# pothosware/PothosComms

Measured on NVIDIA B200. Metric: FIR Msamples/s (cf32, 256 taps) at 1/2/4/8 B200; % HBM roofline; vs host CPU, higher is better.
Workload: dtype f32

## Files before the change

pothoscomms_b200/csrc/fir_os.cu:

```cuda
#include <algorithm>
#include <cmath>
#include <complex>
#include <cstdlib>
#include <vector>

#include "bulk.cuh"
#include "fft.hpp"
#include "os64_core.cuh"

namespace b200c {

struct FirOs64Args {
    const void *in;
    void *out;
    const void *hf;
    const void *twa;
    const void *twb;
    const void *twf;
    long long n_in;
    long long n_out;
    long long in_stride, out_stride;
    int nchan;
    int K;
    int parts;
};

template <bool CONJ, bool SLOT_REV>
__device__ __forceinline__ void step_twiddle(c2 (&v)[64], const c2 *__restrict__ twa, const c2 *__restrict__ twb, const int t)
{
    c2 A[8], B[8];
#pragma unroll
    for (int i = 1; i < 8; i++) { A[i] = twa[i * 64 + t]; B[i] = twb[i * 64 + t]; }
#pragma unroll
    for (int a = 0; a < 8; a++)
#pragma unroll
        for (int b = 0; b < 8; b++) {
            const int j = 8 * a + b, r = SLOT_REV ? rev64(j) : j;
            if (a) v[r] = cmul_p<CONJ>(v[r], A[a]);
            if (b) v[r] = cmul_p<CONJ>(v[r], B[b]);
        }
}

constexpr int kBulkElems = 4098;

template <int MINB>
__global__ void __launch_bounds__(64, MINB) fir_os64_kernel(const FirOs64Args a)
{
    __shared__ __align__(16) c2 F[kOs64SmemElems];
    __shared__ __align__(8) unsigned long long bar;
    const int t = threadIdx.x;
    const c2 *__restrict__ twa = static_cast<const c2 *>(a.twa);
    const c2 *__restrict__ twb = static_cast<const c2 *>(a.twb);
    const int Km1 = a.K - 1;
    const int hop = 4096 - Km1;
    const long long nblk = (a.n_out + hop - 1) / hop;
    const long long tstep = gridDim.x, dch = tstep / nblk, dblk = tstep - dch * nblk;
    long long ch = (long long)blockIdx.x / nblk, blk = (long long)blockIdx.x - ch * nblk;
    auto bulk_src = [&](long long ch, long long blk, const c2 *&src) {
        if (ch >= a.nchan) return false;
        const long long base = blk * hop;
        const c2 *in = static_cast<const c2 *>(a.in) + ch * a.in_stride;
        const int mis = (int)(((reinterpret_cast<unsigned long long>(in) >> 3) + base) & 1);
        src = in + (base - mis);
        return base - mis >= 0 && base - mis + kBulkElems <= a.n_in;
    };
    if (t == 0) mbar_init(&bar, 1);
    __syncthreads();
    const c2 *src = nullptr;
    bool pending = bulk_src(ch, blk, src);
    if (pending && t == 0) bulk_load(F, src, kBulkElems * (unsigned)sizeof(c2), &bar);
    unsigned parity = 0;

    while (ch < a.nchan) {
        const long long base = blk * hop;
        long long nch = ch + dch, nblkpos = blk + dblk;
        if (nblkpos >= nblk) { nblkpos -= nblk; nch++; }
        const c2 *__restrict__ in = static_cast<const c2 *>(a.in) + ch * a.in_stride;
        const c2 *__restrict__ hf = static_cast<const c2 *>(a.hf) + ch * 4096;
        c2 *__restrict__ out = static_cast<c2 *>(a.out) + ch * a.out_stride;
        c2 v[64];
        if (pending) {
            const int mis = (int)(((reinterpret_cast<unsigned long long>(in) >> 3) + base) & 1);
            mbar_wait(&bar, parity);
            parity ^= 1;
#pragma unroll
            for (int n1 = 0; n1 < 64; n1++) v[rev64(n1)] = F[mis + 64 * n1 + t];
        } else {
#pragma unroll
            for (int n1 = 0; n1 < 64; n1++) {
                const long long g = base + 64 * n1 + t;
                v[rev64(n1)] = g < a.n_in ? __ldcg(in + g) : 0ull;
            }
        }
        dft64_dit<false>(v);
        step_twiddle<false, false>(v, twa, twb, t);
        __syncthreads();
#pragma unroll
        for (int k1 = 0; k1 < 64; k1++) F[k1 * kOs64Stride + t] = v[k1];
        __syncthreads();
#pragma unroll
        for (int n2 = 0; n2 < 64; n2++) v[rev64(n2)] = F[t * kOs64Stride + n2];
        dft64_dit<false>(v);
#pragma unroll
        for (int k2 = 0; k2 < 64; k2++) v[k2] = cmul_p<false>(v[k2], hf[64 * k2 + t]);
        dft64_dif<true>(v);
        step_twiddle<true, true>(v, twa, twb, t);
        __syncthreads();
#pragma unroll
        for (int n2 = 0; n2 < 64; n2++) F[t * kOs64Stride + n2] = v[rev64(n2)];
        __syncthreads();
#pragma unroll
        for (int k1 = 0; k1 < 64; k1++) v[k1] = F[k1 * kOs64Stride + t];
        __syncthreads();
        pending = bulk_src(nch, nblkpos, src);
        if (pending && t == 0) bulk_load(F, src, kBulkElems * (unsigned)sizeof(c2), &bar);
        dft64_dif<true>(v);
        c2 *o = out + (base - Km1);
        if (base + hop <= a.n_out) {
#pragma unroll
            for (int n1 = 0; n1 < 64; n1++) {
                const int i = 64 * n1 + t;
                if (i >= Km1) __stcg(o + i, v[rev64(n1)]);
            }
        } else {
#pragma unroll
            for (int n1 = 0; n1 < 64; n1++) {
                const int i = 64 * n1 + t;
                if (i >= Km1 && base + i - Km1 < a.n_out) __stcg(o + i, v[rev64(n1)]);
            }
        }
        ch = nch; blk = nblkpos;
    }
}

constexpr int kOs64Groups = 4;
__global__ void __launch_bounds__(64 * kOs64Groups, 1) fir_os64p_kernel(const FirOs64Args a)
{
    extern __shared__ __align__(16) c2 os64p_dyn[];
    __shared__ __align__(8) unsigned long long bars[kOs64Groups];
    const int g = threadIdx.x >> 6, t = threadIdx.x & 63;
    c2 *F = os64p_dyn + g * kOs64SmemElems;
    c2 *TW = os64p_dyn + kOs64Groups * kOs64SmemElems;
    c2 *HF = TW + 4096;
    unsigned long long *bar = &bars[g];
    auto gsync = [&] { asm volatile("bar.sync %0, 64;" ::"r"(g + 1) : "memory"); };
    const int Km1 = a.K - 1;
    const int hop = 4096 - Km1;
    const long long nblk = (a.n_out + hop - 1) / hop;
    const long long parts = a.parts, ntask = (long long)a.nchan * parts;
    const long long bstep = parts * kOs64Groups;
    auto bulk_src = [&](long long ch, long long blk, const c2 *&src) {
        if (ch >= a.nchan || blk >= nblk) return false;
        const long long base = blk * hop;
        const c2 *in = static_cast<const c2 *>(a.in) + ch * a.in_stride;
        const int mis = (int)(((reinterpret_cast<unsigned long long>(in) >> 3) + base) & 1);
        src = in + (base - mis);
        return base - mis >= 0 && base - mis + kBulkElems <= a.n_in;
    };
    long long task = blockIdx.x;
    if (t == 0) mbar_init(bar, 1);
    gsync();
    const c2 *src = nullptr;
    bool pending = task < ntask && bulk_src(task / parts, (task % parts) * kOs64Groups + g, src);
    if (pending && t == 0) bulk_load(F, src, kBulkElems * (unsigned)sizeof(c2), bar);
    unsigned parity = 0;
    {
        const c2 *__restrict__ twf = static_cast<const c2 *>(a.twf);
        for (int i = threadIdx.x; i < 4096; i += 64 * kOs64Groups) TW[i] = twf[i];
    }
    long long staged = -1;
    for (; task < ntask; task += gridDim.x) {
        const long long ch = task / parts, first = (task - ch * parts) * kOs64Groups + g;
        if (ch != staged) {
            const c2 *__restrict__ hfg = static_cast<const c2 *>(a.hf) + ch * 4096;
            for (int i = threadIdx.x; i < 4096; i += 64 * kOs64Groups) HF[i] = __ldg(hfg + i);
            staged = ch;
        }
        __syncthreads();
        const c2 *__restrict__ in = static_cast<const c2 *>(a.in) + ch * a.in_stride;
        c2 *__restrict__ out = static_cast<c2 *>(a.out) + ch * a.out_stride;
        for (long long blk = first; blk < nblk; blk += bstep) {
            const long long base = blk * hop;
            c2 v[64];
            if (pending) {
                const int mis = (int)(((reinterpret_cast<unsigned long long>(in) >> 3) + base) & 1);
                mbar_wait(bar, parity);
                parity ^= 1;
#pragma unroll
                for (int n1 = 0; n1 < 64; n1++) v[rev64(n1)] = F[mis + 64 * n1 + t];
            } else {
#pragma unroll
                for (int n1 = 0; n1 < 64; n1++) {
                    const long long gi = base + 64 * n1 + t;
                    v[rev64(n1)] = gi < a.n_in ? __ldcg(in + gi) : 0ull;
                }
            }
            dft64_dit<false>(v);
#pragma unroll
            for (int k1 = 1; k1 < 64; k1++) v[k1] = cmul_p<false>(v[k1], TW[k1 * 64 + t]);
            gsync();
#pragma unroll
            for (int k1 = 0; k1 < 64; k1++) F[k1 * kOs64Stride + t] = v[k1];
            gsync();
#pragma unroll
            for (int n2 = 0; n2 < 64; n2++) v[rev64(n2)] = F[t * kOs64Stride + n2];
            dft64_dit<false>(v);
#pragma unroll
            for (int k2 = 0; k2 < 64; k2++) v[k2] = cmul_p<false>(v[k2], HF[64 * k2 + t]);
            dft64_dif<true>(v);
#pragma unroll
            for (int n2 = 1; n2 < 64; n2++) v[rev64(n2)] = cmul_p<true>(v[rev64(n2)], TW[n2 * 64 + t]);
            gsync();
#pragma unroll
            for (int n2 = 0; n2 < 64; n2++) F[t * kOs64Stride + n2] = v[rev64(n2)];
            gsync();
#pragma unroll
            for (int k1 = 0; k1 < 64; k1++) v[k1] = F[k1 * kOs64Stride + t];
            gsync();
            {
                const bool last = blk + bstep >= nblk;
                const long long nt = task + gridDim.x;
                pending = last ? (nt < ntask && bulk_src(nt / parts, (nt % parts) * kOs64Groups + g, src)) : bulk_src(ch, blk + bstep, src);
                if (pending && t == 0) bulk_load(F, src, kBulkElems * (unsigned)sizeof(c2), bar);
            }
            dft64_dif<true>(v);
            c2 *o = out + (base - Km1);
            if (base + hop <= a.n_out) {
#pragma unroll
                for (int n1 = 0; n1 < 64; n1++) {
                    const int i = 64 * n1 + t;
                    if (i >= Km1) __stcg(o + i, v[rev64(n1)]);
                }
            } else {
#pragma unroll
                for (int n1 = 0; n1 < 64; n1++) {
                    const int i = 64 * n1 + t;
                    if (i >= Km1 && base + i - Km1 < a.n_out) __stcg(o + i, v[rev64(n1)]);
                }
            }
        }
        __syncthreads();
    }
}


constexpr bool kOs32PartialTwiddles = false;

template <bool CONJ, bool SLOT_REV>
__device__ __forceinline__ void twiddle32(c2 (&v)[32], const c2 *__restrict__ tw, const int t)
{
    c2 A[8], B[4];
#pragma unroll
    for (int a = 1; a < 8; a++) A[a] = tw[(4 * a) * 32 + t];
#pragma unroll
    for (int b = 1; b < 4; b++) B[b] = tw[b * 32 + t];
#pragma unroll
    for (int k = 1; k < 32; k++) {
        const int a = k >> 2, b = k & 3, r = SLOT_REV ? rev32(k) : k;
        if (a) v[r] = cmul_p<CONJ>(v[r], A[a]);
        if (b) v[r] = cmul_p<CONJ>(v[r], B[b]);
    }
}

struct FirOs32Args {
    const void *in;
    void *out;
    const void *hf;
    const void *tw;
    long long n_in, n_out;
    long long in_stride, out_stride;
    int nchan;
    int K;
    int spread;
    int pdl;
};

constexpr int kOs32Landing = 1032;
template <int WARPS, int MINB, bool TABS = false, bool PT = kOs32PartialTwiddles, bool EARLY = false>
__global__ void __launch_bounds__(32 * WARPS, MINB) fir_os32_kernel(const FirOs32Args a)
{
    extern __shared__ __align__(16) c2 os32_dyn[];
    __shared__ __align__(16) c2 Fs[TABS ? 1 : WARPS][TABS ? 1 : kOs32SmemElems];
    __shared__ __align__(8) unsigned long long bars[WARPS];
    const int t = threadIdx.x & 31, w = threadIdx.x >> 5;
    c2 *F = TABS ? os32_dyn + w * kOs32SmemElems : Fs[TABS ? 0 : w];
    unsigned long long *bar = &bars[w];
    const c2 *__restrict__ tw = static_cast<const c2 *>(a.tw);
    const c2 *__restrict__ hf_tab = nullptr;
    c2 *Lb = F;
    if constexpr (TABS && EARLY) Lb = os32_dyn + WARPS * kOs32SmemElems + 2048 + w * kOs32Landing;
    const int Km1 = a.K - 1;
    const int hop = 1024 - Km1;
    const long long nblk = (a.n_out + hop - 1) / hop;
    const long long tstep = (long long)gridDim.x * WARPS, dch = tstep / nblk, dblk = tstep - dch * nblk;
    const long long task0 = a.spread ? (long long)w * gridDim.x + blockIdx.x : (long long)blockIdx.x * WARPS + w;
    long long ch = task0 / nblk, blk = task0 - ch * nblk;
    constexpr int kBulk = 1026;
    auto bulk_src = [&](long long ch, long long blk, const c2 *&src) {
        if (ch >= a.nchan) return false;
        const long long base = blk * hop;
        const c2 *in = static_cast<const c2 *>(a.in) + ch * a.in_stride;
        const int mis = (int)(((reinterpret_cast<unsigned long long>(in) >> 3) + base) & 1);
        src = in + (base - mis);
        return base - mis >= 0 && base - mis + kBulk <= a.n_in;
    };
    if (t == 0) mbar_init(bar, 1);
    __syncwarp();
    const c2 *src = nullptr;
    bool pending = bulk_src(ch, blk, src);
    unsigned parity = 0;
    if constexpr (TABS) {
        asm volatile("griddepcontrol.launch_dependents;");
        c2 *tab = os32_dyn + WARPS * kOs32SmemElems;
        const c2 *__restrict__ hf0 = static_cast<const c2 *>(a.hf);
        if (a.pdl) {
            for (int i = threadIdx.x; i < 1024; i += 32 * WARPS) { tab[i] = hf0[i]; tab[1024 + i] = tw[i]; }
            asm volatile("griddepcontrol.wait;" ::: "memory");
            if (pending && t == 0) bulk_load(Lb, src, kBulk * (unsigned)sizeof(c2), bar);
        } else {
            if (pending && t == 0) bulk_load(Lb, src, kBulk * (unsigned)sizeof(c2), bar);
            for (int i = threadIdx.x; i < 1024; i += 32 * WARPS) { tab[i] = hf0[i]; tab[1024 + i] = tw[i]; }
        }
        __syncthreads();
        hf_tab = tab; tw = tab + 1024;
    } else {
        if (pending && t == 0) bulk_load(Lb, src, kBulk * (unsigned)sizeof(c2), bar);
    }
    while (ch < a.nchan) {
        const long long base = blk * hop;
        long long nch = ch + dch, nblkpos = blk + dblk;
        if (nblkpos >= nblk) { nblkpos -= nblk; nch++; }
        const c2 *__restrict__ in = static_cast<const c2 *>(a.in) + ch * a.in_stride;
        const c2 *__restrict__ hf = TABS ? hf_tab : static_cast<const c2 *>(a.hf) + ch * 1024;
        c2 *__restrict__ out = static_cast<c2 *>(a.out) + ch * a.out_stride;
        c2 v[32];
        if (pending) {
            const int mis = (int)(((reinterpret_cast<unsigned long long>(in) >> 3) + base) & 1);
            mbar_wait(bar, parity);
            parity ^= 1;
#pragma unroll
            for (int n1 = 0; n1 < 32; n1++) v[rev32(n1)] = Lb[mis + 32 * n1 + t];
        } else {
#pragma unroll
            for (int n1 = 0; n1 < 32; n1++) {
                const long long g = base + 32 * n1 + t;
                v[rev32(n1)] = g < a.n_in ? __ldcg(in + g) : 0ull;
            }
        }
        if constexpr (TABS && EARLY) {
            __syncwarp();
            pending = bulk_src(nch, nblkpos, src);
            if (pending && t == 0) bulk_load(Lb, src, kBulk * (unsigned)sizeof(c2), bar);
        }
        dft32_dit<false>(v);
        if constexpr (PT) twiddle32<false, false>(v, tw, t);
        else {
#pragma unroll
            for (int k1 = 1; k1 < 32; k1++) v[k1] = cmul_p<false>(v[k1], tw[k1 * 32 + t]);
        }
        __syncwarp();
#pragma unroll
        for (int k1 = 0; k1 < 32; k1++) F[k1 * kOs32Stride + t] = v[k1];
        __syncwarp();
#pragma unroll
        for (int n2 = 0; n2 < 32; n2++) v[rev32(n2)] = F[t * kOs32Stride + n2];
        dft32_dit<false>(v);
#pragma unroll
        for (int k2 = 0; k2 < 32; k2++) v[k2] = cmul_p<false>(v[k2], hf[32 * k2 + t]);
        dft32_dif<true>(v);
        if constexpr (PT) twiddle32<true, true>(v, tw, t);
        else {
#pragma unroll
            for (int n2 = 1; n2 < 32; n2++) v[rev32(n2)] = cmul_p<true>(v[rev32(n2)], tw[n2 * 32 + t]);
        }
        __syncwarp();
#pragma unroll
        for (int n2 = 0; n2 < 32; n2++) F[t * kOs32Stride + n2] = v[rev32(n2)];
        __syncwarp();
#pragma unroll
        for (int k1 = 0; k1 < 32; k1++) v[k1] = F[k1 * kOs32Stride + t];
        if constexpr (!(TABS && EARLY)) {
            __syncwarp();
            pending = bulk_src(nch, nblkpos, src);
            if (pending && t == 0) bulk_load(F, src, kBulk * (unsigned)sizeof(c2), bar);
        }
        dft32_dif<true>(v);
        c2 *o = out + (base - Km1);
        if (base + hop <= a.n_out) {
#pragma unroll
            for (int n1 = 0; n1 < 32; n1++) {
                const int i = 32 * n1 + t;
                if (i >= Km1) __stcg(o + i, v[rev32(n1)]);
            }
        } else {
#pragma unroll
            for (int n1 = 0; n1 < 32; n1++) {
                const int i = 32 * n1 + t;
                if (i >= Km1 && base + i - Km1 < a.n_out) __stcg(o + i, v[rev32(n1)]);
            }
        }
        ch = nch; blk = nblkpos;
    }
}

B200C_HD constexpr float cos48(int e)
{
    constexpr float t[48] = {
        1.0f, 0.9914448857307434f, 0.9659258127212524f, 0.9238795042037964f, 0.8660253882408142f, 0.7933533191680908f,
        0.7071067690849304f, 0.6087614297866821f, 0.5f, 0.3826834261417389f, 0.258819043636322f, 0.13052618503570557f, 0.0f,
        -0.13052618503570557f, -0.258819043636322f, -0.3826834261417389f, -0.5f, -0.6087614297866821f, -0.7071067690849304f,
        -0.7933533191680908f, -0.8660253882408142f, -0.9238795042037964f, -0.9659258127212524f, -0.9914448857307434f, -1.0f,
        -0.9914448857307434f, -0.9659258127212524f, -0.9238795042037964f, -0.8660253882408142f, -0.7933533191680908f,
        -0.7071067690849304f, -0.6087614297866821f, -0.5f, -0.3826834261417389f, -0.258819043636322f, -0.13052618503570557f, 0.0f,
        0.13052618503570557f, 0.258819043636322f, 0.3826834261417389f, 0.5f, 0.6087614297866821f, 0.7071067690849304f,
        0.7933533191680908f, 0.8660253882408142f, 0.9238795042037964f, 0.9659258127212524f, 0.9914448857307434f};
    return t[e % 48];
}
B200C_HD constexpr float sin48(int e) { return cos48(e + 36); }

B200C_HD constexpr int rev16(int k) { return 4 * (k & 3) + (k >> 2); }
template <bool INV> B200C_HD void dft16_dif(c2 (&x)[16])
{
#pragma unroll
    for (int k = 0; k < 4; k++) {
        dft4_p<INV>(x[k], x[k + 4], x[k + 8], x[k + 12]);
        x[k + 4] = mul_w64<INV>(x[k + 4], 4 * k);
        x[k + 8] = mul_w64<INV>(x[k + 8], 8 * k);
        x[k + 12] = mul_w64<INV>(x[k + 12], 12 * k);
    }
#pragma unroll
    for (int g = 0; g < 4; g++) dft4_p<INV>(x[4 * g], x[4 * g + 1], x[4 * g + 2], x[4 * g + 3]);
}

B200C_HD c2 cmul_acc(c2 f, c2 w, c2 acc)
{
    float fx, fy, wx, wy;
    upk(f, fx, fy); upk(w, wx, wy);
    return fma2(f, pk(wx, wx), fma2(pk(-fy, fx), pk(wy, wy), acc));
}

struct FirOsX32Args {
    const void *in;
    void *out;
    const void *hx;
    const void *tw;
    const void *tw3;
    long long n_in, n_out;
    long long p0;
    int m0;
    int pdl;
};
constexpr int kX32Rows = 48, kX32SmemElems = kX32Rows * kOs32Stride;

constexpr int kX32TabElems = 3072 + 1536 + 1024;
template <int WARPS, int MINB, bool PT = false, bool SPLIT = false>
__global__ void __launch_bounds__(32 * WARPS, MINB) fir_os32x_kernel(const FirOsX32Args a)
{
    extern __shared__ __align__(16) c2 x32_smem[];
    __shared__ __align__(8) unsigned long long bars[WARPS];
    const int t = threadIdx.x & 31, wp = threadIdx.x >> 5;
    const c2 *__restrict__ tw = static_cast<const c2 *>(a.tw);
    const c2 *__restrict__ tw3 = static_cast<const c2 *>(a.tw3);
    const c2 *__restrict__ hx = static_cast<const c2 *>(a.hx);
    c2 *F = x32_smem + wp * kX32SmemElems;
    c2 *const Lb = F;
    unsigned long long &bar = bars[wp];
    const c2 *__restrict__ in = static_cast<const c2 *>(a.in);
    c2 *__restrict__ out = static_cast<c2 *>(a.out);
    const int m0 = a.m0, hop_out = 1536 - m0, hop_in = hop_out / 3 * 2;
    const long long nblk = (a.n_out + hop_out - 1) / hop_out;
    constexpr int kBulk = 1026;
    auto bulk_src = [&](long long blk, const c2 *&src) {
        if (blk >= nblk) return false;
        const long long P = a.p0 + blk * hop_in;
        const int mis = (int)(((reinterpret_cast<unsigned long long>(in) >> 3) + (unsigned long long)P) & 1);
        src = in + (P - mis);
        return P - mis >= 0 && P - mis + kBulk <= a.n_in;
    };
    if (t == 0) mbar_init(&bar, 1);
    __syncwarp();
    long long blk = (long long)blockIdx.x * WARPS + wp;
    const long long bstep = (long long)gridDim.x * WARPS;
    const c2 *src = nullptr;
    bool pending = bulk_src(blk, src);
    unsigned parity = 0;
    if constexpr (WARPS > 1) {
        asm volatile("griddepcontrol.launch_dependents;");
        c2 *tab = x32_smem + WARPS * kX32SmemElems;
        auto stage = [&] {
            for (int i = threadIdx.x; i < 3072; i += 32 * WARPS) tab[i] = hx[i];
            for (int i = threadIdx.x; i < 1536; i += 32 * WARPS) tab[3072 + i] = tw3[i];
            for (int i = threadIdx.x; i < 1024; i += 32 * WARPS) tab[3072 + 1536 + i] = tw[i];
        };
        if (a.pdl) {
            stage();
            asm volatile("griddepcontrol.wait;" ::: "memory");
            if (pending && t == 0) bulk_load(Lb, src, kBulk * (unsigned)sizeof(c2), &bar);
        } else {
            if (pending && t == 0) bulk_load(Lb, src, kBulk * (unsigned)sizeof(c2), &bar);
            stage();
        }
        __syncthreads();
        hx = tab; tw3 = tab + 3072; tw = tab + 3072 + 1536;
    } else {
        if (pending && t == 0) bulk_load(Lb, src, kBulk * (unsigned)sizeof(c2), &bar);
    }
    for (; blk < nblk; blk += bstep) {
        const long long P = a.p0 + blk * hop_in;
        c2 v[32];
        if (pending) {
            const int mis = (int)(((reinterpret_cast<unsigned long long>(in) >> 3) + (unsigned long long)P) & 1);
            mbar_wait(&bar, parity);
            parity ^= 1;
#pragma unroll
            for (int n1 = 0; n1 < 32; n1++) v[rev32(n1)] = Lb[mis + 32 * n1 + t];
        } else {
#pragma unroll
            for (int n1 = 0; n1 < 32; n1++) {
                const long long g = P + 32 * n1 + t;
                v[rev32(n1)] = (g >= 0 && g < a.n_in) ? __ldcg(in + g) : 0ull;
            }
        }
        dft32_dit<false>(v);
        if constexpr (PT) twiddle32<false, false>(v, tw, t);
        else {
#pragma unroll
            for (int k1 = 1; k1 < 32; k1++) v[k1] = cmul_p<false>(v[k1], tw[k1 * 32 + t]);
        }
        __syncwarp();
#pragma unroll
        for (int k1 = 0; k1 < 32; k1++) F[k1 * kOs32Stride + t] = v[k1];
        __syncwarp();
#pragma unroll
        for (int n2 = 0; n2 < 32; n2++) v[rev32(n2)] = F[t * kOs32Stride + n2];
        dft32_dit<false>(v);
        c2 s[3][16];
#pragma unroll
        for (int c = 0; c < 16; c++) {
            const c2 xa = v[c], xb = v[c + 16];
            const c2 h0 = hx[32 * c + t], g0 = hx[1536 + 32 * c + t];
            const c2 h1 = hx[32 * (c + 16) + t], g1 = hx[1536 + 32 * (c + 16) + t];
            const c2 h2 = hx[32 * (c + 32) + t], g2 = hx[1536 + 32 * (c + 32) + t];
            s[c % 3][c / 3] = cmul_acc(xb, g0, cmul_p<false>(xa, h0));
            s[(c + 16) % 3][(c + 16) / 3] = cmul_acc(xa, g1, cmul_p<false>(xb, h1));
            s[(c + 32) % 3][(c + 32) / 3] = cmul_acc(xb, g2, cmul_p<false>(xa, h2));
        }
#pragma unroll
        for (int c1 = 0; c1 < 3; c1++) dft16_dif<true>(s[c1]);
        __syncwarp();
        c2 twb1 = 0, twb2 = 0;
        if constexpr (PT) { twb1 = tw3[16 * 32 + t]; twb2 = tw3[32 * 32 + t]; }
#pragma unroll
        for (int v2 = 0; v2 < 16; v2++) {
            const int r = rev16(v2);
            const c2 a0 = s[0][r];
            const c2 a1 = v2 ? cmul_s(s[1][r], cos48(v2), sin48(v2)) : s[1][r];
            const c2 a2 = v2 ? cmul_s(s[2][r], cos48(2 * v2), sin48(2 * v2)) : s[2][r];
            const c2 t1 = add2(a1, a2);
            const c2 t2 = fma2(t1, pk(-0.5f, -0.5f), a0);
            const c2 t3 = rot_p<true>(mul2(sub2(a1, a2), pk(0.8660254037844386f, 0.8660254037844386f)));
            const c2 y0 = add2(a0, t1), y1 = add2(t2, t3), y2 = sub2(t2, t3);
            if constexpr (PT) {
                const c2 wa = v2 ? tw3[v2 * 32 + t] : pk(1.f, 0.f);
                F[v2 * kOs32Stride + t] = v2 ? cmul_p<false>(y0, wa) : y0;
                F[(16 + v2) * kOs32Stride + t] = cmul_p<false>(y1, v2 ? cmul_p<false>(wa, twb1) : twb1);
                F[(32 + v2) * kOs32Stride + t] = cmul_p<false>(y2, v2 ? cmul_p<false>(wa, twb2) : twb2);
            } else {
                F[v2 * kOs32Stride + t] = v2 ? cmul_p<false>(y0, tw3[v2 * 32 + t]) : y0;
                F[(16 + v2) * kOs32Stride + t] = cmul_p<false>(y1, tw3[(16 + v2) * 32 + t]);
                F[(32 + v2) * kOs32Stride + t] = cmul_p<false>(y2, tw3[(32 + v2) * 32 + t]);
            }
        }
        __syncwarp();
        const long long mbase = blk * hop_out - m0;
        const bool whole = (blk + 1) * (long long)hop_out <= a.n_out;
        c2 *const o = out + mbase + t;
        const int d0 = t - m0;
        const int left = whole ? 0x7fffffff : (int)(a.n_out - mbase) - t;
#pragma unroll
        for (int k1 = 0; k1 < 32; k1++) v[rev32(k1)] = F[t * kOs32Stride + k1];
        if constexpr (SPLIT) {
            __syncwarp();
            pending = bulk_src(blk + bstep, src);
            if (pending && t == 0) bulk_load(F, src, kBulk * (unsigned)sizeof(c2), &bar);
        }
        dft32_dit<true>(v);
        if (whole) {
#pragma unroll
            for (int n1 = 0; n1 < 32; n1++)
                if (d0 + 48 * n1 >= 0) __stcg(o + 48 * n1, v[n1]);
        } else {
#pragma unroll
            for (int n1 = 0; n1 < 32; n1++)
                if (d0 + 48 * n1 >= 0 && 48 * n1 < left) __stcg(o + 48 * n1, v[n1]);
        }
        if constexpr (SPLIT) {
            const int tt = t & 15, h = t >> 4;
            c2 x[16];
#pragma unroll
            for (int j = 0; j < 16; j++) x[j] = F[(32 + tt) * kOs32Stride + 2 * j + h];
            __syncwarp();
            dft16_dif<true>(x);
            c2 *const o2 = out + mbase + tt + 32 + 48 * 16 * h;
            const int d2 = tt - m0 + 32 + 48 * 16 * h;
            const int left2 = whole ? 0x7fffffff : (int)(a.n_out - mbase) - tt - 32 - 48 * 16 * h;
#pragma unroll
            for (int m = 0; m < 16; m++) {
                const c2 mine = h ? mul_w64<true>(x[rev16(m)], 2 * m) : x[rev16(m)];
                const c2 other = __shfl_xor_sync(0xffffffffu, mine, 16);
                const c2 y = h ? sub2(other, mine) : add2(mine, other);
                if (d2 + 48 * m >= 0 && 48 * m < left2) __stcg(o2 + 48 * m, y);
            }
            continue;
        }
        if (t < 16) {
#pragma unroll
            for (int k1 = 0; k1 < 32; k1++) v[rev32(k1)] = F[(32 + t) * kOs32Stride + k1];
        }
        __syncwarp();
        pending = bulk_src(blk + bstep, src);
        if (pending && t == 0) bulk_load(F, src, kBulk * (unsigned)sizeof(c2), &bar);
        if (t < 16) {
            dft32_dit<true>(v);
            if (whole) {
#pragma unroll
                for (int n1 = 0; n1 < 32; n1++)
                    if (d0 + 48 * n1 + 32 >= 0) __stcg(o + 48 * n1 + 32, v[n1]);
            } else {
#pragma unroll
                for (int n1 = 0; n1 < 32; n1++)
                    if (d0 + 48 * n1 + 32 >= 0 && 48 * n1 + 32 < left) __stcg(o + 48 * n1 + 32, v[n1]);
            }
        }
    }
}

struct FirOs32RArgs {
    const float *in;
    float *out;
    const void *hf;
    const void *tw;
    long long n_in, n_out;
    int K;
};

template <int WARPS, int MINB, bool EARLY = false>
__global__ void __launch_bounds__(32 * WARPS, MINB) fir_os32r_kernel(const FirOs32RArgs a)
{
    extern __shared__ __align__(16) c2 os32r_dyn[];
    __shared__ __align__(8) unsigned long long bars[WARPS];
    const int t = threadIdx.x & 31, wp = threadIdx.x >> 5;
    c2 *F = os32r_dyn + wp * kOs32SmemElems;
    c2 *Lb = (WARPS > 1 && EARLY) ? os32r_dyn + WARPS * kOs32SmemElems + 2048 + wp * kOs32Landing : F;
    unsigned long long &bar = bars[wp];
    const float *Ff = reinterpret_cast<const float *>(Lb);
    const c2 *__restrict__ tw = static_cast<const c2 *>(a.tw);
    const c2 *__restrict__ hf = static_cast<const c2 *>(a.hf);
    if constexpr (WARPS > 1) {
        c2 *tab = os32r_dyn + WARPS * kOs32SmemElems;
        for (int i = threadIdx.x; i < 1024; i += 32 * WARPS) { tab[i] = hf[i]; tab[1024 + i] = tw[i]; }
        __syncthreads();
        hf = tab; tw = tab + 1024;
    }
    const int Km1 = a.K - 1, hop = 1024 - Km1;
    const long long npair = (a.n_out + 2LL * hop - 1) / (2LL * hop);
    auto bulk_src = [&](long long bp, const float *&src, int &mis, unsigned &bytes) {
        if (bp >= npair) return false;
        const long long base = bp * 2LL * hop;
        mis = (int)(((reinterpret_cast<unsigned long long>(a.in) >> 2) + base) & 3);
        const int count = (mis + hop + 1024 + 3) & ~3;
        src = a.in + (base - mis);
        bytes = (unsigned)count * 4u;
        return base - mis >= 0 && base - mis + count <= a.n_in;
    };
    if (t == 0) mbar_init(&bar, 1);
    __syncwarp();
    long long bp = (long long)blockIdx.x * WARPS + wp;
    const float *src = nullptr;
    int mis = 0, mis_next = 0;
    unsigned bytes = 0;
    bool pending = bulk_src(bp, src, mis, bytes);
    if (pending && t == 0) bulk_load(Lb, src, bytes, &bar);
    unsigned parity = 0;
    while (bp < npair) {
        const long long base = bp * 2LL * hop, nbp = bp + (long long)gridDim.x * WARPS;
        c2 v[32];
        if (pending) {
            mbar_wait(&bar, parity);
            parity ^= 1;
#pragma unroll
            for (int n1 = 0; n1 < 32; n1++) v[rev32(n1)] = pk(Ff[mis + 32 * n1 + t], Ff[mis + hop + 32 * n1 + t]);
        } else {
#pragma unroll
            for (int n1 = 0; n1 < 32; n1++) {
                const long long ga = base + 32 * n1 + t, gb = ga + hop;
                v[rev32(n1)] = pk(ga < a.n_in ? __ldg(a.in + ga) : 0.f, gb < a.n_in ? __ldg(a.in + gb) : 0.f);
            }
        }
        if constexpr (WARPS > 1 && EARLY) {
            __syncwarp();
            pending = bulk_src(nbp, src, mis_next, bytes);
            if (pending && t == 0) bulk_load(Lb, src, bytes, &bar);
        }
        dft32_dit<false>(v);
// ... 458 lines not shown
    std::vector<float> H(2 * (size_t)L * M * N);
    for (size_t sub = 0; sub < gp.size(); sub++) {
        host_fft(gp[sub]);
        for (int f = 0; f < N; f++) {
            H[2 * (sub * N + f)] = (float)(gp[sub][f].real() / N);
            H[2 * (sub * N + f) + 1] = (float)(gp[sub][f].imag() / N);
        }
    }
    if (p.d_H && p.H_floats < H.size()) { cudaFree(p.d_H); p.d_H = nullptr; }
    int rc;
    if ((rc = upload(&p.d_H, H))) return rc;
    p.H_floats = std::max(p.H_floats, H.size());
    if (!p.d_tw1k) {
        std::vector<float> tb;
        unit_root_table(tb, 1024, 32, 32, 1);
        if ((rc = upload(&p.d_tw1k, tb))) return rc;
    }
    p.general = true; p.real = real_data;
    p.N = N; p.M = (int)M; p.L = (int)L;
    p.hopq = (int)(N - span);
    p.start0 = (K - 1) + a_min * (long long)M;
    p.K = (int)K;
    p.ready = true;
    return B200C_OK;
}

int fir_os_configure(FirOsPlan &p, int dtype, const double *taps, size_t ntaps, bool complex_taps, size_t M, size_t L,
                     bool force)
{
    p.ready = false; p.general = false; p.real = false; p.osp = false; p.real32 = false; p.x32 = false;
    const bool no_x32 = [] { const char *e = std::getenv("B200C_OSX"); return e && std::atoi(e) == 0; }();
    if (dtype == B200C_CF32 && L == 3 && M == 2 && !no_x32 && ntaps >= 2 && ntaps <= 1200 &&
        (force || (ntaps + L - 1) / L >= kFirOsAutoMinTapsX32)) {
        const long long K = (long long)((ntaps + L - 1) / L);
        int m0 = (int)((ntaps - 2 + 1) / 2);
        m0 = (m0 + 2) / 3 * 3;
        const double two_pi = 2.0 * 3.14159265358979323846264338327950288;
        std::vector<float> hx(2 * 3072), tb(2 * 48 * 32);
        for (int k = 0; k < 3072; k++) {
            std::complex<double> acc(0.0, 0.0);
            for (size_t tt = 0; tt < ntaps; tt++) {
                const std::complex<double> h = complex_taps ? std::complex<double>(taps[2 * tt], taps[2 * tt + 1]) : std::complex<double>(taps[tt], 0.0);
                const long long e = ((long long)k * (long long)tt) % 3072;
                acc += h * std::polar(1.0, -two_pi * (double)e / 3072.0);
            }
            acc *= std::polar(1.0 / 3072.0, two_pi * (double)k / 3072.0);
            hx[2 * k] = (float)acc.real();
            hx[2 * k + 1] = (float)acc.imag();
        }
        for (int n2 = 0; n2 < 48; n2++)
            for (int t = 0; t < 32; t++) {
                tb[2 * (n2 * 32 + t)] = (float)std::cos(two_pi * (double)(n2 * t) / 1536.0);
                tb[2 * (n2 * 32 + t) + 1] = (float)std::sin(two_pi * (double)(n2 * t) / 1536.0);
            }
        int rc;
        if ((rc = upload(&p.d_hx, hx))) return rc;
        if ((rc = upload(&p.d_tw3, tb))) return rc;
        if (!p.d_tw1k) {
            unit_root_table(tb, 1024, 32, 32, 1);
            if ((rc = upload(&p.d_tw1k, tb))) return rc;
        }
        p.N = 1024; p.K = (int)K; p.M = 2; p.L = 3; p.m0 = m0; p.p0 = (K - 1) - 2 * (long long)(m0 / 3);
        p.x32 = true;
        p.ready = true;
        return B200C_OK;
    }
    if (dtype == B200C_CF32 && M == 1 && L == 1) {
        if (ntaps < 2 || ntaps > kFirOsMaxTaps || (!force && ntaps < kFirOsAutoMinTapsFloat)) return B200C_OK;
        std::vector<float> tb, hf;
        int rc;
        p.N = pick_length(ntaps);
        if (p.N == 4096) {
            if (!p.d_twa) {
                unit_root_table(tb, 4096, 8, 64, 8);
                if ((rc = upload(&p.d_twa, tb))) return rc;
                unit_root_table(tb, 4096, 8, 64, 1);
                if ((rc = upload(&p.d_twb, tb))) return rc;
                unit_root_table(tb, 4096, 64, 64, 1);
                if ((rc = upload(&p.d_twf, tb))) return rc;
            }
            taps_spectrum(hf, 4096, taps, ntaps, complex_taps);
            if ((rc = upload(&p.d_hf, hf))) return rc;
        } else {
            if (!p.d_tw1k) {
                unit_root_table(tb, 1024, 32, 32, 1);
                if ((rc = upload(&p.d_tw1k, tb))) return rc;
            }
            taps_spectrum(hf, 1024, taps, ntaps, complex_taps);
            if ((rc = upload(&p.d_hf1k, hf))) return rc;
        }
        p.K = (int)ntaps;
        p.ready = true;
        return B200C_OK;
    }
    if (dtype == B200C_F32 && M == 1 && L == 1 && !complex_taps && ntaps >= (force ? 2 : kFirOsAutoMinTapsFloat) && ntaps <= kFirOs1kMaxTaps &&
        !(std::getenv("B200C_OS32R") && std::atoi(std::getenv("B200C_OS32R")) == 0)) {
        std::vector<float> tb, hf;
        int rc;
        if (!p.d_tw1k) {
            unit_root_table(tb, 1024, 32, 32, 1);
            if ((rc = upload(&p.d_tw1k, tb))) return rc;
        }
        taps_spectrum(hf, 1024, taps, ntaps, false);
        if ((rc = upload(&p.d_hf1k, hf))) return rc;
        p.N = 1024; p.K = (int)ntaps; p.real32 = true;
        p.ready = true;
        return B200C_OK;
    }
    const bool osp = dtype == B200C_CF32 && L <= 4 && M <= 4 && std::max(L, M) >= 2 && !(L == 1 && M <= 2) &&
                     !(std::getenv("B200C_OSP") && std::atoi(std::getenv("B200C_OSP")) == 0);
    if ((dtype == B200C_CF32 || dtype == B200C_F32) && (M <= 2 || osp) && L <= (force ? kFirOsGenForcedMaxInterp : kFirOsGenMaxInterp)) {
        const size_t per_phase = (ntaps + L - 1) / L;
        static const bool no_group = [] { const char *e = std::getenv("B200C_OSPG"); return e && std::atoi(e) == 0; }();
        const int nw = (int)std::max(L, M), G = nw == 2 ? 6 : nw == 3 ? 4 : 3;
        const bool grouped = osp && !no_group &&
                             sizeof(c2) * ((size_t)L * M * 1024 + 1024 + G * ((size_t)M * kOs32SmemElems + (size_t)L * osp_plane_stride((int)L))) <= 227 * 1024;
        const size_t min_taps = (M == 1 && L == 1) ? kFirOsAutoMinTapsReal
                                : (osp && M == 4 && L == 1) ? kFirOsAutoMinTapsOspDecim4
                                : osp ? kFirOsAutoMinTapsOsp
                                : L >= 5 ? kFirOsAutoMinTapsWideInterp : kFirOsAutoMinTapsResamp;
        if (!force && per_phase < min_taps) return B200C_OK;
        if (ntaps < 2) return B200C_OK;
        p.osp = osp;
        p.ospg = 0;
        const int rc = configure_general(p, dtype == B200C_F32, taps, ntaps, complex_taps, M, L);
        if (rc == B200C_OK && p.ready && grouped) p.ospg = G;
        return rc;
    }
    return B200C_OK;
}

void fir_os_destroy(FirOsPlan &p)
{
    for (void **d : {&p.d_hf, &p.d_twa, &p.d_twb, &p.d_twf, &p.d_hf1k, &p.d_tw1k, &p.d_H, &p.d_hx, &p.d_tw3}) {
        if (*d) cudaFree(*d);
        *d = nullptr;
    }
    p.H_floats = 0;
    p.ready = false;
}

const char *fir_os_kernel_name(const FirOsPlan &p)
{
    if (p.x32) return "fir_os32x_kernel";
    if (p.general) return p.osp ? (p.ospg ? "fir_ospg_kernel" : "fir_osp_kernel") : "fir_os32g_kernel";
    if (p.real32) return "fir_os32r_kernel";
    return p.N == 1024 ? "fir_os32_kernel" : "fir_os64p_kernel";
}

template <int M, bool MULTI_L, bool REAL, bool TILE_OUT, int MINB>
static int launch_general(const FirOs32GArgs &a, long long nblk, int sm_count, cudaStream_t stream)
{
    auto kern = fir_os32g_kernel<M, MULTI_L, REAL, TILE_OUT, MINB>;
    const size_t smem = sizeof(c2) * (size_t)osg_smem_elems(a.L, TILE_OUT);
    static thread_local bool configured[16] = {false};
    int dev = 0;
    B200C_CUDA_TRY(cudaGetDevice(&dev));
    if (dev < 16 && !configured[dev]) {
        B200C_CUDA_TRY(cudaFuncSetAttribute(kern, cudaFuncAttributeMaxDynamicSharedMemorySize, 64 * 1024));
        configured[dev] = true;
    }
    const long long by_smem = std::max<long long>(1, (220 * 1024) / (long long)(smem + 1024));
    const int per_sm = (int)std::min<long long>(MINB, by_smem);
    const int grid = (int)std::min<long long>(nblk, (long long)sm_count * per_sm * 4);
    kern<<<grid, 32, smem, stream>>>(a);
    B200C_CUDA_TRY(cudaGetLastError());
    return B200C_OK;
}

template <int NW, int MINB>
static void launch_osp(const FirOs32GArgs &a, int M, size_t smem, long long nblk, int sm_count, cudaStream_t stream)
{
    auto kern = fir_osp_kernel<NW, MINB>;
    static thread_local bool configured[16] = {false};
    int dev = 0;
    if (cudaGetDevice(&dev) == cudaSuccess && dev < 16 && !configured[dev]) {
        cudaFuncSetAttribute(kern, cudaFuncAttributeMaxDynamicSharedMemorySize, 100 * 1024);
        if (const char *e = std::getenv("B200C_OSP_CARVE")) cudaFuncSetAttribute(kern, cudaFuncAttributePreferredSharedMemoryCarveout, std::atoi(e));
        configured[dev] = true;
    }
    static const int forced = [] { const char *e = std::getenv("B200C_OSP_PERSM"); return e ? std::atoi(e) : 0; }();
    const long long per_sm = std::max<long long>(1, std::min<long long>(forced > 0 ? forced : MINB, (224 * 1024) / (long long)(smem + 1024)));
    const int grid = (int)std::min<long long>(nblk, (long long)sm_count * per_sm * 2);
    kern<<<grid, 32 * NW, smem, stream>>>(a, M);
}

template <int NW, int G>
static void launch_ospg(const FirOs32GArgs &a, int M, size_t smem, long long nblk, int sm_count, cudaStream_t stream)
{
    auto kern = fir_ospg_kernel<NW, G>;
    static thread_local bool configured[16] = {false};
    int dev = 0;
    if (cudaGetDevice(&dev) == cudaSuccess && dev < 16 && !configured[dev]) {
        cudaFuncSetAttribute(kern, cudaFuncAttributeMaxDynamicSharedMemorySize, 227 * 1024);
        configured[dev] = true;
    }
    const int grid = (int)std::min<long long>((nblk + G - 1) / G, (long long)sm_count);
    kern<<<grid, 32 * NW * G, smem, stream>>>(a, M);
}

static bool pdl_enabled()
{
    static const bool on = [] { const char *e = std::getenv("B200C_PDL"); return !e || std::atoi(e) != 0; }();
    return on;
}
template <typename Kernel, typename Args>
static cudaError_t launch_dependent(Kernel kern, int grid, int block, size_t smem, cudaStream_t stream, const Args &a)
{
    cudaLaunchConfig_t cfg = {};
    cfg.gridDim = dim3((unsigned)grid); cfg.blockDim = dim3((unsigned)block); cfg.dynamicSmemBytes = smem; cfg.stream = stream;
    cudaLaunchAttribute attr[1];
    attr[0].id = cudaLaunchAttributeProgrammaticStreamSerialization;
    attr[0].val.programmaticStreamSerializationAllowed = 1;
    cfg.attrs = attr; cfg.numAttrs = 1;
    return cudaLaunchKernelEx(&cfg, kern, a);
}

bool fir_os_batchable(const FirOsPlan &p) { return p.ready && !p.x32 && !p.general && !p.real32; }

int fir_os_launch(const FirOsPlan &p, const void *d_in, size_t in_elems, void *d_out, size_t nq, int sm_count,
                  cudaStream_t stream, const FirOsBatch *batch)
{
    if (nq == 0) return B200C_OK;
    if (batch && !fir_os_batchable(p)) { set_error("filter bank: the batched launch serves complex float32 L = M = 1 only"); return B200C_ERR_UNSUPPORTED; }
    const int nchan = batch ? batch->nchan : 1;
    if (p.x32) {
        FirOsX32Args a;
        a.in = d_in; a.out = d_out; a.hx = p.d_hx; a.tw = p.d_tw1k; a.tw3 = p.d_tw3;
        a.n_in = (long long)in_elems; a.n_out = (long long)nq * 3; a.p0 = p.p0; a.m0 = p.m0;
        const long long nblk = (a.n_out + (1536 - p.m0) - 1) / (1536 - p.m0);
        const size_t tile = sizeof(c2) * kX32SmemElems;
        const size_t smem = 12 * tile + sizeof(c2) * kX32TabElems;
        static thread_local bool configured[16] = {false};
        int dev = 0;
        B200C_CUDA_TRY(cudaGetDevice(&dev));
        if (dev < 16 && !configured[dev]) {
            B200C_CUDA_TRY(cudaFuncSetAttribute(fir_os32x_kernel<12, 1, true, true>, cudaFuncAttributeMaxDynamicSharedMemorySize, (int)smem));
            configured[dev] = true;
        }
        const int grid = (int)std::min<long long>((nblk + 11) / 12, (long long)sm_count);
        a.pdl = pdl_enabled() ? 1 : 0;
        if (a.pdl) B200C_CUDA_TRY(launch_dependent(fir_os32x_kernel<12, 1, true, true>, grid, 32 * 12, smem, stream, a));
        else fir_os32x_kernel<12, 1, true, true><<<grid, 32 * 12, smem, stream>>>(a);
        B200C_CUDA_TRY(cudaGetLastError());
        return B200C_OK;
    }
    if (p.general) {
        FirOs32GArgs a;
        a.in = d_in; a.out = d_out; a.H = p.d_H; a.tw = p.d_tw1k;
        a.n_in = (long long)in_elems; a.nq = (long long)nq; a.start0 = p.start0; a.L = p.L; a.hop = p.hopq;
        if (p.osp) {
            const int nw = std::max(p.L, p.M);
            const size_t smem = sizeof(c2) * ((size_t)p.M * kOs32SmemElems + (size_t)p.L * osp_plane_stride(p.L));
            const long long nblk = ((long long)nq + p.hopq - 1) / p.hopq;
            const size_t shared_tab = sizeof(c2) * ((size_t)p.L * p.M * 1024 + 1024);
            if (p.ospg && nw == 3) launch_ospg<3, 4>(a, p.M, shared_tab + 4 * smem, nblk, sm_count, stream);
            else if (p.ospg && nw == 2) launch_ospg<2, 6>(a, p.M, shared_tab + 6 * smem, nblk, sm_count, stream);
            else if (p.ospg && nw == 4) launch_ospg<4, 3>(a, p.M, shared_tab + 3 * smem, nblk, sm_count, stream);
            else if (nw == 2) launch_osp<2, 7>(a, p.M, smem, nblk, sm_count, stream);
            else if (nw == 3) launch_osp<3, 5>(a, p.M, smem, nblk, sm_count, stream);
            else launch_osp<4, 3>(a, p.M, smem, nblk, sm_count, stream);
            B200C_CUDA_TRY(cudaGetLastError());
            return B200C_OK;
        }
        const long long per = (long long)p.hopq * (p.real ? 2 : 1);
        const long long nblk = ((long long)nq + per - 1) / per;
        const bool ml = p.L > 1, tile = p.L >= 2 && p.L <= 4;
#define OSG(MM, RR, MB1, MBL)                                                                                      \
    (!ml ? launch_general<MM, false, RR, false, MB1>(a, nblk, sm_count, stream)                                      \
         : tile ? launch_general<MM, true, RR, true, MBL>(a, nblk, sm_count, stream)                                 \
                : launch_general<MM, true, RR, false, MBL>(a, nblk, sm_count, stream))
        if (p.M == 1) return p.real ? OSG(1, true, 12, 10) : OSG(1, false, 12, 10);
        return p.real ? OSG(2, true, 10, 8) : OSG(2, false, 10, 8);
#undef OSG
    }
    if (p.real32) {
        FirOs32RArgs a;
        a.in = static_cast<const float *>(d_in); a.out = static_cast<float *>(d_out); a.hf = p.d_hf1k; a.tw = p.d_tw1k;
        a.n_in = (long long)in_elems; a.n_out = (long long)nq; a.K = p.K;
        const long long npair = ((long long)nq + p.hop() - 1) / p.hop();
        const size_t tile = sizeof(c2) * kOs32SmemElems;
        const size_t smem_early = 12 * tile + sizeof(c2) * 2048 + sizeof(c2) * 12 * kOs32Landing;
        static thread_local bool configured[16] = {false};
        int dev = 0;
        B200C_CUDA_TRY(cudaGetDevice(&dev));
        if (dev < 16 && !configured[dev]) {
            B200C_CUDA_TRY(cudaFuncSetAttribute(fir_os32r_kernel<12, 1, true>, cudaFuncAttributeMaxDynamicSharedMemorySize, (int)smem_early));
            configured[dev] = true;
        }
        const int grid = (int)std::min<long long>((npair + 11) / 12, (long long)sm_count);
        fir_os32r_kernel<12, 1, true><<<grid, 32 * 12, smem_early, stream>>>(a);
        B200C_CUDA_TRY(cudaGetLastError());
        return B200C_OK;
    }
    const size_t n_out = nq;
    const long long nblk = (((long long)n_out + p.hop() - 1) / p.hop()) * nchan;
    if (p.N == 1024) {
        FirOs32Args a;
        a.in = d_in; a.out = d_out; a.hf = batch ? batch->d_hf : p.d_hf1k; a.tw = p.d_tw1k;
        a.n_in = (long long)in_elems; a.n_out = (long long)n_out; a.K = p.K;
        a.nchan = nchan; a.in_stride = batch ? batch->in_stride : 0; a.out_stride = batch ? batch->out_stride : 0;
        a.spread = 0; a.pdl = 0;
        if (nchan == 1) {
            const size_t smem_early = sizeof(c2) * (12 * (size_t)kOs32SmemElems + 2048 + 12 * (size_t)kOs32Landing);
            static thread_local bool configured[16] = {false};
            int dev = 0;
            B200C_CUDA_TRY(cudaGetDevice(&dev));
            if (dev < 16 && !configured[dev]) {
                B200C_CUDA_TRY(cudaFuncSetAttribute(fir_os32_kernel<12, 1, true, false, true>, cudaFuncAttributeMaxDynamicSharedMemorySize, (int)smem_early));
                configured[dev] = true;
            }
            a.spread = nblk < 12LL * sm_count ? 1 : 0;
            const int grid = (int)std::min<long long>(a.spread ? nblk : (nblk + 11) / 12, (long long)sm_count);
            a.pdl = pdl_enabled() ? 1 : 0;
            if (a.pdl) B200C_CUDA_TRY(launch_dependent(fir_os32_kernel<12, 1, true, false, true>, grid, 32 * 12, smem_early, stream, a));
            else fir_os32_kernel<12, 1, true, false, true><<<grid, 32 * 12, smem_early, stream>>>(a);
            B200C_CUDA_TRY(cudaGetLastError());
            return B200C_OK;
        }
        {
            const int grid = (int)std::min<long long>(nblk, (long long)sm_count * 12 * 4);
            fir_os32_kernel<1, 12><<<grid, 32, 0, stream>>>(a);
        }
        B200C_CUDA_TRY(cudaGetLastError());
        return B200C_OK;
    }
    FirOs64Args a;
    a.in = d_in; a.out = d_out; a.hf = batch ? batch->d_hf : p.d_hf; a.twa = p.d_twa; a.twb = p.d_twb; a.twf = p.d_twf;
    a.n_in = (long long)in_elems; a.n_out = (long long)n_out; a.K = p.K;
    a.nchan = nchan; a.in_stride = batch ? batch->in_stride : 0; a.out_stride = batch ? batch->out_stride : 0;
    a.parts = 1;
    static const bool persistent = [] { const char *e = std::getenv("B200C_OS64P"); return !e || std::atoi(e) != 0; }();
    const long long blocks_per_chan = ((long long)n_out + p.hop() - 1) / p.hop();
    if (persistent && (long long)nchan * blocks_per_chan >= 4LL * kOs64Groups * sm_count) {
        const size_t smem = sizeof(c2) * ((size_t)kOs64Groups * kOs64SmemElems + 4096 + 4096);
        if (nchan == 1) a.parts = sm_count;
        else {
            const long long maxp = std::max<long long>(1, blocks_per_chan / 16);
            double best = -1.0;
            for (long long q = 1; q <= std::min<long long>(maxp, 32); q++) {
                const long long T = (long long)nchan * q, rounds = (T + sm_count - 1) / sm_count;
                const double util = (double)T / (double)(rounds * sm_count) - 1.5e-3 * (double)(q - 1);
                if (util > best) { best = util; a.parts = (int)q; }
            }
        }
        static thread_local bool configured[16] = {false};
        int dev = 0;
        B200C_CUDA_TRY(cudaGetDevice(&dev));
        if (dev < 16 && !configured[dev]) {
            B200C_CUDA_TRY(cudaFuncSetAttribute(fir_os64p_kernel, cudaFuncAttributeMaxDynamicSharedMemorySize, (int)smem));
            configured[dev] = true;
        }
        fir_os64p_kernel<<<sm_count, 64 * kOs64Groups, smem, stream>>>(a);
        B200C_CUDA_TRY(cudaGetLastError());
        return B200C_OK;
    }
    const int grid = (int)std::min<long long>(nblk, (long long)sm_count * 4 * 4);
    fir_os64_kernel<4><<<grid, 64, 0, stream>>>(a);
    B200C_CUDA_TRY(cudaGetLastError());
    return B200C_OK;
}

}
```

Baseline: 301,700.

## Keep FFT twiddle and filter-spectrum tables in tensor memory instead of shared memory

For the single-channel table-staged 1024-point overlap-save kernel, twiddles and the filter spectrum now live in Blackwell tensor memory (TMEM). Each CTA allocates 128 TMEM columns, and four warps fill them, one per lane quarter. The per-element shared-memory table reads in the twiddle and filter-multiply stages become tcgen05.ld loads of eight complex values at a time. This aims to cut shared-memory bandwidth pressure and frees 16 KB of dynamic shared memory, at the cost of TMEM allocation and fences and extra ld-wait latency in each block. The per-thread table mapping depends on warp index modulo 4, which looks right only if every warp's lane mapping matches its TMEM lane quarter.

```diff
diff --git a/pothoscomms_b200/csrc/fir_os.cu b/pothoscomms_b200/csrc/fir_os.cu
--- a/pothoscomms_b200/csrc/fir_os.cu
+++ b/pothoscomms_b200/csrc/fir_os.cu
@@ -275,6 +275,33 @@
     int pdl;
 };
 
+constexpr unsigned kOs32TmemCols = 128;
+__device__ __forceinline__ void tmem_ld_c2x8(unsigned taddr, c2 (&v)[8])
+{
+    unsigned r[16];
+    asm volatile("tcgen05.ld.sync.aligned.32x32b.x16.b32 {%0, %1, %2, %3, %4, %5, %6, %7, %8, %9, %10, %11, %12, %13, %14, %15}, [%16];\n\t"
+                 "tcgen05.wait::ld.sync.aligned;"
+                 : "=r"(r[0]), "=r"(r[1]), "=r"(r[2]), "=r"(r[3]), "=r"(r[4]), "=r"(r[5]), "=r"(r[6]), "=r"(r[7]), "=r"(r[8]),
+                   "=r"(r[9]), "=r"(r[10]), "=r"(r[11]), "=r"(r[12]), "=r"(r[13]), "=r"(r[14]), "=r"(r[15])
+                 : "r"(taddr)
+                 : "memory");
+#pragma unroll
+    for (int j = 0; j < 8; j++) v[j] = pk(__uint_as_float(r[2 * j]), __uint_as_float(r[2 * j + 1]));
+}
+__device__ __forceinline__ void tmem_st_c2x8(unsigned taddr, const c2 (&v)[8])
+{
+    unsigned r[16];
+#pragma unroll
+    for (int j = 0; j < 8; j++) {
+        float x, y;
+        upk(v[j], x, y);
+        r[2 * j] = __float_as_uint(x); r[2 * j + 1] = __float_as_uint(y);
+    }
+    asm volatile("tcgen05.st.sync.aligned.32x32b.x16.b32 [%0], {%1, %2, %3, %4, %5, %6, %7, %8, %9, %10, %11, %12, %13, %14, %15, %16};"
+                 ::"r"(taddr), "r"(r[0]), "r"(r[1]), "r"(r[2]), "r"(r[3]), "r"(r[4]), "r"(r[5]), "r"(r[6]), "r"(r[7]), "r"(r[8]),
+                   "r"(r[9]), "r"(r[10]), "r"(r[11]), "r"(r[12]), "r"(r[13]), "r"(r[14]), "r"(r[15])
+                 : "memory");
+}
 constexpr int kOs32Landing = 1032;
 template <int WARPS, int MINB, bool TABS = false, bool PT = kOs32PartialTwiddles, bool EARLY = false>
 __global__ void __launch_bounds__(32 * WARPS, MINB) fir_os32_kernel(const FirOs32Args a)
@@ -286,9 +313,10 @@
     c2 *F = TABS ? os32_dyn + w * kOs32SmemElems : Fs[TABS ? 0 : w];
     unsigned long long *bar = &bars[w];
     const c2 *__restrict__ tw = static_cast<const c2 *>(a.tw);
-    const c2 *__restrict__ hf_tab = nullptr;
+    __shared__ unsigned tmem_base_s;
+    unsigned tq = 0;
     c2 *Lb = F;
-    if constexpr (TABS && EARLY) Lb = os32_dyn + WARPS * kOs32SmemElems + 2048 + w * kOs32Landing;
+    if constexpr (TABS && EARLY) Lb = os32_dyn + WARPS * kOs32SmemElems + w * kOs32Landing;
     const int Km1 = a.K - 1;
     const int hop = 1024 - Km1;
     const long long nblk = (a.n_out + hop - 1) / hop;
@@ -311,18 +339,40 @@
     unsigned parity = 0;
     if constexpr (TABS) {
         asm volatile("griddepcontrol.launch_dependents;");
-        c2 *tab = os32_dyn + WARPS * kOs32SmemElems;
+        static_assert(WARPS >= 4, "the tables are written by four warps, one per TMEM lane quarter");
+        if (w == 0) {
+            asm volatile("tcgen05.alloc.cta_group::1.sync.aligned.shared::cta.b32 [%0], %1;" ::"r"(smem_u32(&tmem_base_s)), "r"(kOs32TmemCols) : "memory");
+            asm volatile("tcgen05.relinquish_alloc_permit.cta_group::1.sync.aligned;" ::: "memory");
+        }
+        asm volatile("tcgen05.fence::before_thread_sync;" ::: "memory");
+        __syncthreads();
+        asm volatile("tcgen05.fence::after_thread_sync;" ::: "memory");
+        tq = tmem_base_s + ((unsigned)(32 * (w & 3)) << 16);
         const c2 *__restrict__ hf0 = static_cast<const c2 *>(a.hf);
+        auto stage = [&] {
+            if (w < 4) {
+#pragma unroll
+                for (int q = 0; q < 4; q++) {
+                    c2 T[8], H[8];
+#pragma unroll
+                    for (int j = 0; j < 8; j++) { T[j] = tw[(8 * q + j) * 32 + t]; H[j] = hf0[32 * (8 * q + j) + t]; }
+                    tmem_st_c2x8(tq + 16 * q, T);
+                    tmem_st_c2x8(tq + 64 + 16 * q, H);
+                }
+                asm volatile("tcgen05.wait::st.sync.aligned;" ::: "memory");
+            }
+        };
         if (a.pdl) {
-            for (int i = threadIdx.x; i < 1024; i += 32 * WARPS) { tab[i] = hf0[i]; tab[1024 + i] = tw[i]; }
+            stage();
             asm volatile("griddepcontrol.wait;" ::: "memory");
             if (pending && t == 0) bulk_load(Lb, src, kBulk * (unsigned)sizeof(c2), bar);
         } else {
             if (pending && t == 0) bulk_load(Lb, src, kBulk * (unsigned)sizeof(c2), bar);
-            for (int i = threadIdx.x; i < 1024; i += 32 * WARPS) { tab[i] = hf0[i]; tab[1024 + i] = tw[i]; }
-        }
+            stage();
+        }
+        asm volatile("tcgen05.fence::before_thread_sync;" ::: "memory");
         __syncthreads();
-        hf_tab = tab; tw = tab + 1024;
+        asm volatile("tcgen05.fence::after_thread_sync;" ::: "memory");
     } else {
         if (pending && t == 0) bulk_load(Lb, src, kBulk * (unsigned)sizeof(c2), bar);
     }
@@ -331,7 +381,7 @@
         long long nch = ch + dch, nblkpos = blk + dblk;
         if (nblkpos >= nblk) { nblkpos -= nblk; nch++; }
         const c2 *__restrict__ in = static_cast<const c2 *>(a.in) + ch * a.in_stride;
-        const c2 *__restrict__ hf = TABS ? hf_tab : static_cast<const c2 *>(a.hf) + ch * 1024;
+        const c2 *__restrict__ hf = static_cast<const c2 *>(a.hf) + ch * 1024;
         c2 *__restrict__ out = static_cast<c2 *>(a.out) + ch * a.out_stride;
         c2 v[32];
         if (pending) {
@@ -353,7 +403,16 @@
             if (pending && t == 0) bulk_load(Lb, src, kBulk * (unsigned)sizeof(c2), bar);
         }
         dft32_dit<false>(v);
-        if constexpr (PT) twiddle32<false, false>(v, tw, t);
+        if constexpr (TABS) {
+#pragma unroll
+            for (int q = 0; q < 4; q++) {
+                c2 T[8];
+                tmem_ld_c2x8(tq + 16 * q, T);
+#pragma unroll
+                for (int j = 0; j < 8; j++)
+                    if (8 * q + j) v[8 * q + j] = cmul_p<false>(v[8 * q + j], T[j]);
+            }
+        } else if constexpr (PT) twiddle32<false, false>(v, tw, t);
         else {
 #pragma unroll
             for (int k1 = 1; k1 < 32; k1++) v[k1] = cmul_p<false>(v[k1], tw[k1 * 32 + t]);
@@ -365,10 +424,29 @@
 #pragma unroll
         for (int n2 = 0; n2 < 32; n2++) v[rev32(n2)] = F[t * kOs32Stride + n2];
         dft32_dit<false>(v);
-#pragma unroll
-        for (int k2 = 0; k2 < 32; k2++) v[k2] = cmul_p<false>(v[k2], hf[32 * k2 + t]);
+        if constexpr (TABS) {
+#pragma unroll
+            for (int q = 0; q < 4; q++) {
+                c2 H[8];
+                tmem_ld_c2x8(tq + 64 + 16 * q, H);
+#pragma unroll
+                for (int j = 0; j < 8; j++) v[8 * q + j] = cmul_p<false>(v[8 * q + j], H[j]);
+            }
+        } else {
+#pragma unroll
+            for (int k2 = 0; k2 < 32; k2++) v[k2] = cmul_p<false>(v[k2], hf[32 * k2 + t]);
+        }
         dft32_dif<true>(v);
-        if constexpr (PT) twiddle32<true, true>(v, tw, t);
+        if constexpr (TABS) {
+#pragma unroll
+            for (int q = 0; q < 4; q++) {
+                c2 T[8];
+                tmem_ld_c2x8(tq + 16 * q, T);
+#pragma unroll
+                for (int j = 0; j < 8; j++)
+                    if (8 * q + j) v[rev32(8 * q + j)] = cmul_p<true>(v[rev32(8 * q + j)], T[j]);
+            }
+        } else if constexpr (PT) twiddle32<true, true>(v, tw, t);
         else {
 #pragma unroll
             for (int n2 = 1; n2 < 32; n2++) v[rev32(n2)] = cmul_p<true>(v[rev32(n2)], tw[n2 * 32 + t]);
@@ -400,6 +478,12 @@
             }
         }
         ch = nch; blk = nblkpos;
+    }
+    if constexpr (TABS) {
+        asm volatile("tcgen05.fence::before_thread_sync;" ::: "memory");
+        __syncthreads();
+        asm volatile("tcgen05.fence::after_thread_sync;" ::: "memory");
+        if (w == 0) asm volatile("tcgen05.dealloc.cta_group::1.sync.aligned.b32 %0, %1;" ::"r"(tmem_base_s), "r"(kOs32TmemCols) : "memory");
     }
 }
 
@@ -1464,7 +1548,7 @@
         a.nchan = nchan; a.in_stride = batch ? batch->in_stride : 0; a.out_stride = batch ? batch->out_stride : 0;
         a.spread = 0; a.pdl = 0;
         if (nchan == 1) {
-            const size_t smem_early = sizeof(c2) * (12 * (size_t)kOs32SmemElems + 2048 + 12 * (size_t)kOs32Landing);
+            const size_t smem_early = sizeof(c2) * (12 * (size_t)kOs32SmemElems + 12 * (size_t)kOs32Landing);
             static thread_local bool configured[16] = {false};
             int dev = 0;
             B200C_CUDA_TRY(cudaGetDevice(&dev));
```

New measurement: 326,700 (median of 6 runs). +8.3%, better.
